# bliunlpr/Robust_e2e_gan

Hardware: AMD Instinct MI355X
Metric: joint_train utterances/sec (higher is better)
Workload: dtype f32; 1 GPU; config4: joint_train.py full GAN+ASR step, B=32 per GPU, T=800, F=257->80, L=40, V=4233, enhancer 2xBLSTM-256, VGG+3xBLSTMP-512, loc-attention decoder 300, D basic ndf64, Adadelta; global_batch=32, per_rank_batch=32, parallelism=dp1, utterance_lengths=560..800 frames (mean 680 of T=800)

## Files before the change

### robust_e2e_gan_amd/csrc/wino_wgrad.hip

```cpp
#include <hip/hip_runtime.h>
#include "../../include/re2e.h"
#include "common.h"

namespace {
typedef float f32x16 __attribute__((ext_vector_type(16)));
typedef float f32x2 __attribute__((ext_vector_type(2)));
constexpr unsigned WW_OOB = 0x80000000u;
constexpr int WW_CB = 64, WW_OB = 32;

struct WwArgs {
  const float* x; const float* dy; float* slabs;
  int NI, H, W, C, Cout;
  int px, py, npatch, nsplit, ncb, nblk;
  unsigned x_bytes, dy_bytes;
  const int* row_lim;
  int flat;
  int dbg;
};

template <int TXW>
__global__ __launch_bounds__(256, 2) void wino_wgrad_kernel(WwArgs p) {
  constexpr int TYH = 32 / TXW, PW = 2 * TXW, PH = 2 * TYH;
  constexpr int XW = PW + 2, XH = PH + 2, XPIX = XW * XH;
  constexpr int XIT = (XPIX * 16 + 255) / 256, DIT = PW * PH * 8 / 256;
  extern __shared__ __attribute__((aligned(16))) float smem[];
  float* xs = smem;
  float* ds = smem + XPIX * WW_CB;
  const int tid = threadIdx.x, lane = tid & 63, lr = lane & 31, lh = lane >> 5;
  const int wid = __builtin_amdgcn_readfirstlane(tid >> 6);
  const int xk = blockIdx.x >> 3;
  const int blk = p.flat ? blockIdx.x % p.nblk : xk % p.nblk, split = p.flat ? blockIdx.x / p.nblk : (xk / p.nblk) * 8 + (blockIdx.x & 7);
  if (split >= p.nsplit) return;
  const int cb = blk % p.ncb, ob = blk / p.ncb;
  const int c0 = cb * WW_CB, o0 = ob * WW_OB;
  const __amdgpu_buffer_rsrc_t rsX = __builtin_amdgcn_make_buffer_rsrc(const_cast<float*>(p.x), 0, p.x_bytes, 0x00020000);
  const __amdgpu_buffer_rsrc_t rsD = __builtin_amdgcn_make_buffer_rsrc(const_cast<float*>(p.dy), 0, p.dy_bytes, 0x00020000);
  const int per = (p.npatch + p.nsplit - 1) / p.nsplit;
  const int pbeg = split * per, pend = min(p.npatch, pbeg + per);

  f32x4 xr[XIT], dr[DIT];
  auto load_patch = [&](int pi) {
    const int n = pi / (p.py * p.px), rem = pi - n * (p.py * p.px);
    const int pyi = rem / p.px, pxi = rem - pyi * p.px;
    const int y0 = pyi * PH, x0 = pxi * PW;
#pragma unroll
    for (int it = 0; it < XIT; ++it) {
      const int item = it * 256 + tid, pix = item >> 4, c4 = item & 15;
      const int yy = pix / XW, xx = pix - yy * XW, iy = y0 - 1 + yy, ix = x0 - 1 + xx;
      const bool ok = pix < XPIX && (unsigned)iy < (unsigned)p.H && (unsigned)ix < (unsigned)p.W;
      const unsigned off = (unsigned)((((n * p.H + iy) * p.W + ix) * p.C + c0 + c4 * 4) * 4);
      xr[it] = __builtin_bit_cast(f32x4, __builtin_amdgcn_raw_buffer_load_b128(rsX, ok ? off : WW_OOB, 0, 0));
    }
#pragma unroll
    for (int it = 0; it < DIT; ++it) {
      const int item = it * 256 + tid, pix = item >> 3, o4 = item & 7;
      const int yy = pix / PW, xx = pix - yy * PW, oy = y0 + yy, ox = x0 + xx;
      const bool ok = oy < p.H && ox < p.W;
      const unsigned off = (unsigned)((((n * p.H + oy) * p.W + ox) * p.Cout + o0 + o4 * 4) * 4);
      dr[it] = __builtin_bit_cast(f32x4, __builtin_amdgcn_raw_buffer_load_b128(rsD, ok ? off : WW_OOB, 0, 0));
    }
  };
  auto store_patch = [&]() {
#pragma unroll
    for (int it = 0; it < XIT; ++it) {
      const int item = it * 256 + tid;
      if (item < XPIX * 16) *reinterpret_cast<f32x4*>(xs + item * 4) = xr[it];
    }
#pragma unroll
    for (int it = 0; it < DIT; ++it) *reinterpret_cast<f32x4*>(ds + (it * 256 + tid) * 4) = dr[it];
  };

  const int rA = wid == 0 ? 0 : (wid == 2 ? 2 : 1), rB = wid == 3 ? 3 : (wid == 2 ? 1 : 2);
  const float sg = wid == 1 ? 1.f : -1.f;
  const float a0 = wid == 3 ? 0.f : 1.f, a1 = wid == 0 ? 0.f : (wid == 1 ? 1.f : -1.f);
  constexpr int HR = TYH / 2;
  const float* xA = xs + ((rA + 2 * HR * lh) * XW) * WW_CB + 2 * lr;
  const float* xB = xs + ((rB + 2 * HR * lh) * XW) * WW_CB + 2 * lr;
  const float* dB = ds + (2 * HR * lh * PW) * WW_OB + lr;

  f32x16 acc[4][2];
#pragma unroll
  for (int j = 0; j < 4; ++j)
#pragma unroll
    for (int ct = 0; ct < 2; ++ct)
#pragma unroll
      for (int r = 0; r < 16; ++r) acc[j][ct][r] = 0.f;

  for (int pi = pbeg; pi < pend; ++pi) {
    if (p.row_lim) {
      const int n = pi / (p.py * p.px), pyi = (pi - n * (p.py * p.px)) / p.px;
      if (pyi * PH >= p.row_lim[n]) continue;
    }
    load_patch(pi);
    store_patch();
    __syncthreads();
    f32x2 t[4], v[2][4];
    float m[2][4];
    auto prep = [&](const int s, f32x2 (&vv)[4], float (&mm)[4]) {
      const int tyl = s / TXW, txl = s % TXW;
#pragma unroll
      for (int j = 0; j < 4; ++j) {
        if (txl != 0 && j < 2) { t[j] = t[j + 2]; continue; }
        const f32x2 da = *reinterpret_cast<const f32x2*>(xA + ((2 * tyl) * XW + 2 * txl + j) * WW_CB);
        const f32x2 db = *reinterpret_cast<const f32x2*>(xB + ((2 * tyl) * XW + 2 * txl + j) * WW_CB);
        t[j] = da + sg * db;
      }
      vv[0] = t[0] - t[2]; vv[1] = t[1] + t[2]; vv[2] = t[2] - t[1]; vv[3] = t[1] - t[3];
      const float e00 = dB[((2 * tyl) * PW + 2 * txl) * WW_OB], e01 = dB[((2 * tyl) * PW + 2 * txl + 1) * WW_OB];
      const float e10 = dB[((2 * tyl + 1) * PW + 2 * txl) * WW_OB], e11 = dB[((2 * tyl + 1) * PW + 2 * txl + 1) * WW_OB];
      const float s0 = a0 * e00 + a1 * e10, s1 = a0 * e01 + a1 * e11;
      mm[0] = s0; mm[1] = s0 + s1; mm[2] = s0 - s1; mm[3] = -s1;
    };
    prep(0, v[0], m[0]);
#pragma unroll
    for (int s = 0; s < 16; ++s) {
      if (s + 1 < 16) prep(s + 1, v[(s + 1) & 1], m[(s + 1) & 1]);
#pragma unroll
      for (int j = 0; j < 4; ++j) {
        acc[j][0] = __builtin_amdgcn_mfma_f32_32x32x2f32(v[s & 1][j][0], m[s & 1][j], acc[j][0], 0, 0, 0);
        acc[j][1] = __builtin_amdgcn_mfma_f32_32x32x2f32(v[s & 1][j][1], m[s & 1][j], acc[j][1], 0, 0, 0);
      }
      if (s + 1 < 16) {
#pragma unroll
        for (int g = 0; g < 8; ++g) {
          __builtin_amdgcn_sched_group_barrier(0x008, 1, 0);
          __builtin_amdgcn_sched_group_barrier(0x100, 1, 0);
          __builtin_amdgcn_sched_group_barrier(0x002, 4, 0);
        }
      }
    }
    __syncthreads();
  }
  float* sl = p.slabs + ((long)split * 16 + 4 * wid) * p.C * p.Cout;
#pragma unroll
  for (int j = 0; j < 4; ++j)
#pragma unroll
    for (int ct = 0; ct < 2; ++ct)
#pragma unroll
      for (int r = 0; r < 16; ++r) {
        const int c = c0 + 2 * ((r & 3) + 8 * (r >> 2) + 4 * lh) + ct;
        sl[((long)j * p.C + c) * p.Cout + o0 + lr] = acc[j][ct][r];
      }
}

#ifdef RE2E_EXPERIMENTS
#include "experiments/wino_wgrad_dma.hip"
#endif

__global__ __launch_bounds__(1024) void wino_wgrad_reduce_kernel(const float* __restrict__ slabs, int nsplit, long tot, float* __restrict__ red) {
  __shared__ float part[16][64];
  const int e = threadIdx.x & 63, sl = threadIdx.x >> 6;
  const long i = (long)blockIdx.x * 64 + e;
  float s = 0.f;
  if (i < tot)
    for (int z = sl; z < nsplit; z += 16) s += slabs[(long)z * tot + i];
  part[sl][e] = s;
  __syncthreads();
  if (sl != 0 || i >= tot) return;
  s = 0.f;
#pragma unroll
  for (int q = 0; q < 16; ++q) s += part[q][e];
  red[i] = s;
}

__global__ __launch_bounds__(256) void wino_wgrad_final_kernel(const float* __restrict__ slabs, int nsplit, int C, int Cout, float* __restrict__ gw,
                                                               float beta) {
  const long i = (long)blockIdx.x * 256 + threadIdx.x;
  const long CO = (long)C * Cout;
  if (i >= CO) return;
  const int o = (int)(i % Cout), c = (int)(i / Cout);
  float u[4][4];
#pragma unroll
  for (int pos = 0; pos < 16; ++pos) u[pos >> 2][pos & 3] = 0.f;
  for (int s = 0; s < nsplit; ++s) {
    const float* sp = slabs + (long)s * 16 * CO + i;
#pragma unroll
    for (int pos = 0; pos < 16; ++pos) u[pos >> 2][pos & 3] += sp[pos * CO];
  }
  float t[3][4];
#pragma unroll
  for (int j = 0; j < 4; ++j) {
    t[0][j] = u[0][j] + 0.5f * (u[1][j] + u[2][j]);
    t[1][j] = 0.5f * (u[1][j] - u[2][j]);
    t[2][j] = 0.5f * (u[1][j] + u[2][j]) + u[3][j];
  }
  float* wp = gw + ((long)o * C + c) * 9;
#pragma unroll
  for (int a = 0; a < 3; ++a) {
    const float r0 = t[a][0] + 0.5f * (t[a][1] + t[a][2]), r1 = 0.5f * (t[a][1] - t[a][2]), r2 = 0.5f * (t[a][1] + t[a][2]) + t[a][3];
    if (beta != 0.f) { wp[a * 3] += r0; wp[a * 3 + 1] += r1; wp[a * 3 + 2] += r2; }
    else { wp[a * 3] = r0; wp[a * 3 + 1] = r1; wp[a * 3 + 2] = r2; }
  }
}

struct WwPlan { bool wide; int px, py, npatch, nsplit, ncb, nblk; size_t bytes; };
WwPlan ww_plan(int NI, int H, int W, int C, int Cout) {
  WwPlan q;
  const long pad_w = (long)cdiv(H, 8) * 8 * cdiv(W, 16) * 16, pad_n = (long)cdiv(H, 16) * 16 * cdiv(W, 8) * 8;
  q.wide = pad_w <= pad_n;
  q.px = cdiv(W, q.wide ? 16 : 8); q.py = cdiv(H, q.wide ? 8 : 16);
  q.npatch = NI * q.py * q.px;
  q.ncb = C / WW_CB; q.nblk = q.ncb * (Cout / WW_OB);
  int s = cdiv(1536, q.nblk);
  if (s > q.npatch / 8) s = q.npatch / 8;
  if (s < 1) s = 1;
  q.nsplit = s;
  q.bytes = (size_t)(s + 1) * 16 * C * Cout * sizeof(float);
  return q;
}

template <int TXW>
void launch_ww(const WwArgs& a, hipStream_t st) {
  constexpr int PW = 2 * TXW, PH = 64 / TXW;
#ifdef RE2E_EXPERIMENTS
  static const bool dma = exp_env("RE2E_WW_DMA") && atoi(exp_env("RE2E_WW_DMA")) == 1;
  if (dma) {
    constexpr size_t lds2 = (size_t)2 * (192 * WW_CB + PW * PH * WW_OB) * sizeof(float);
    static LdsLimit lim2;
    lim2.ensure(reinterpret_cast<const void*>(&wino_wgrad_dma_kernel<TXW>), lds2);
    hipLaunchKernelGGL((wino_wgrad_dma_kernel<TXW>), dim3((unsigned)(cdiv(a.nsplit, 8) * 8 * a.nblk)), dim3(256), lds2, st, a);
    return;
  }
#endif
  constexpr size_t lds = (size_t)((PW + 2) * (PH + 2) * WW_CB + PW * PH * WW_OB) * sizeof(float);
  static LdsLimit lim;
  lim.ensure(reinterpret_cast<const void*>(&wino_wgrad_kernel<TXW>), lds);
  hipLaunchKernelGGL((wino_wgrad_kernel<TXW>), dim3((unsigned)(cdiv(a.nsplit, 8) * 8 * a.nblk)), dim3(256), lds, st, a);
}
}

extern "C" size_t re2e_conv3x3_wino_wgrad_workspace_bytes(int NI, int H, int W, int C, int Cout) {
  if (NI <= 0 || H <= 0 || W <= 0 || C <= 0 || Cout <= 0 || C % WW_CB || Cout % WW_OB) return 0;
  return ww_plan(NI, H, W, C, Cout).bytes;
}

static int ww_impl(const float* in, int NI, int H, int W, int C, const float* dout, int Cout, float* gw, float beta, const int* row_lim, void* workspace,
                   size_t workspace_bytes, hipStream_t stream) {
  RE2E_CHECK_ARG(in && dout && gw && workspace, "null operand");
  RE2E_CHECK_ARG(NI > 0 && H > 0 && W > 0 && C > 0 && Cout > 0, "bad geometry");
  RE2E_CHECK_ARG(beta == 0.f || beta == 1.f, "beta must be 0 or 1");
  if (C % WW_CB || Cout % WW_OB) { re2e_set_error("re2e_conv3x3_wino_wgrad: C must be a multiple of 64 and Cout of 32 (got %d, %d)", C, Cout); return RE2E_EUNSUPPORTED; }
  const long x_bytes = (long)NI * H * W * C * 4, dy_bytes = (long)NI * H * W * Cout * 4;
  if (x_bytes >= 0x7FFFFF00L || dy_bytes >= 0x7FFFFF00L) { re2e_set_error("re2e_conv3x3_wino_wgrad: tensors must be < 2 GiB"); return RE2E_EUNSUPPORTED; }
  RE2E_CHECK_ARG((reinterpret_cast<uintptr_t>(in) & 15) == 0 && (reinterpret_cast<uintptr_t>(dout) & 15) == 0, "in / dout must be 16-byte aligned");
  const WwPlan q = ww_plan(NI, H, W, C, Cout);
  RE2E_CHECK_ARG(workspace_bytes >= q.bytes, "workspace too small (re2e_conv3x3_wino_wgrad_workspace_bytes)");
  WwArgs a;
  a.x = in; a.dy = dout; a.slabs = static_cast<float*>(workspace);
  a.NI = NI; a.H = H; a.W = W; a.C = C; a.Cout = Cout;
  a.px = q.px; a.py = q.py; a.npatch = q.npatch; a.nsplit = q.nsplit; a.ncb = q.ncb; a.nblk = q.nblk;
  a.x_bytes = (unsigned)x_bytes; a.dy_bytes = (unsigned)dy_bytes;
  a.row_lim = row_lim;
  a.dbg = exp_env("RE2E_WW_DBG") ? atoi(exp_env("RE2E_WW_DBG")) : 0;
  a.flat = exp_env("RE2E_WW_FLAT") ? atoi(exp_env("RE2E_WW_FLAT")) : 0;
  static const bool log_calls = getenv("RE2E_IGEMM_LOG") != nullptr;
  if (log_calls)
    fprintf(stderr, "[igemm] A=WinoW B=DenseM tile=64x32x2 vec=1 M=%d N=%d K=%ld splits=%d\n", 9 * C, Cout, (long)NI * H * W, q.nsplit);
  if (q.wide) launch_ww<8>(a, stream); else launch_ww<4>(a, stream);
  const long tot = 16L * C * Cout;
  float* red = a.slabs + (long)q.nsplit * tot;
  hipLaunchKernelGGL(wino_wgrad_reduce_kernel, dim3((unsigned)cdiv(tot, 64)), dim3(1024), 0, stream, a.slabs, q.nsplit, tot, red);
  hipLaunchKernelGGL(wino_wgrad_final_kernel, dim3((unsigned)cdiv((long)C * Cout, 256)), dim3(256), 0, stream, red, 1, C, Cout, gw, beta);
  RE2E_LAUNCH_CHECK();
  return RE2E_OK;
}

extern "C" int re2e_conv3x3_wino_wgrad(const float* in, int NI, int H, int W, int C, const float* dout, int Cout, float* gw, float beta, void* workspace,
                                       size_t workspace_bytes, hipStream_t stream) {
  return ww_impl(in, NI, H, W, C, dout, Cout, gw, beta, nullptr, workspace, workspace_bytes, stream);
}

extern "C" int re2e_conv3x3_wino_wgrad_rows(const float* in, int NI, int H, int W, int C, const float* dout, int Cout, float* gw, float beta,
                                            const int* row_lim, void* workspace, size_t workspace_bytes, hipStream_t stream) {
  RE2E_CHECK_ARG(row_lim, "null row limits");
  return ww_impl(in, NI, H, W, C, dout, Cout, gw, beta, row_lim, workspace, workspace_bytes, stream);
}
```

Baseline: 686.9 utterances/s.

## Widen Winograd wgrad tile to two output blocks, balance valid patches, fuse reductions

The Winograd weight-gradient kernel now gives each block two 32-wide output-channel blocks (NOB=2). This reuses the transformed input across twice the MFMAs and adds register prefetch of the next patch into the main loop. Split ranges are now computed over valid patches only, following the row limits, so padded rows no longer leave splits unbalanced. The separate reduce and final kernels are merged into one finish kernel, and slab stores use buffer stores. The cost is more register pressure: occupancy bound drops to one block per SIMD, and the split-count heuristic changes.

```diff
diff --git a/robust_e2e_gan_amd/csrc/experiments/wino_wgrad_deep.hip b/robust_e2e_gan_amd/csrc/experiments/wino_wgrad_deep.hip
--- /dev/null
+++ b/robust_e2e_gan_amd/csrc/experiments/wino_wgrad_deep.hip
@@ -0,0 +1,61 @@
+template <int TXW, int NOB>
+__device__ __forceinline__ void ww_products_deep(const float* xA, const float* xB, const float* dB, const float sg, const float a0, const float a1,
+                                                 f32x16 (&acc)[NOB][4][2]) {
+  constexpr int TYH = 32 / TXW, PW = 2 * TXW, XW = PW + 2, OBW = WW_OB * NOB;
+  f32x2 t[4], v[2][4];
+  float m[2][NOB][4];
+  struct Raw { f32x2 a[4], b[4]; float e[NOB][4]; };
+  auto fetch = [&](const int s, Raw& w) {
+    const int tyl = s / TXW, txl = s % TXW;
+#pragma unroll
+    for (int j = 0; j < 4; ++j) {
+      if (txl != 0 && j < 2) continue;
+      w.a[j] = *reinterpret_cast<const f32x2*>(xA + ((2 * tyl) * XW + 2 * txl + j) * WW_CB);
+      w.b[j] = *reinterpret_cast<const f32x2*>(xB + ((2 * tyl) * XW + 2 * txl + j) * WW_CB);
+    }
+#pragma unroll
+    for (int nb = 0; nb < NOB; ++nb) {
+      const float* dn = dB + nb * WW_OB;
+      w.e[nb][0] = dn[((2 * tyl) * PW + 2 * txl) * OBW]; w.e[nb][1] = dn[((2 * tyl) * PW + 2 * txl + 1) * OBW];
+      w.e[nb][2] = dn[((2 * tyl + 1) * PW + 2 * txl) * OBW]; w.e[nb][3] = dn[((2 * tyl + 1) * PW + 2 * txl + 1) * OBW];
+    }
+  };
+  auto xform = [&](const int s, const Raw& w, f32x2 (&vv)[4], float (&mm)[NOB][4]) {
+    const int txl = s % TXW;
+#pragma unroll
+    for (int j = 0; j < 4; ++j) {
+      if (txl != 0 && j < 2) { t[j] = t[j + 2]; continue; }
+      t[j] = w.a[j] + sg * w.b[j];
+    }
+    vv[0] = t[0] - t[2]; vv[1] = t[1] + t[2]; vv[2] = t[2] - t[1]; vv[3] = t[1] - t[3];
+#pragma unroll
+    for (int nb = 0; nb < NOB; ++nb) {
+      const float s0 = a0 * w.e[nb][0] + a1 * w.e[nb][2], s1 = a0 * w.e[nb][1] + a1 * w.e[nb][3];
+      mm[nb][0] = s0; mm[nb][1] = s0 + s1; mm[nb][2] = s0 - s1; mm[nb][3] = -s1;
+    }
+  };
+  Raw w[2];
+  fetch(0, w[0]);
+  fetch(1, w[1]);
+  xform(0, w[0], v[0], m[0]);
+#pragma unroll
+  for (int s = 0; s < 16; ++s) {
+    if (s + 1 < 16) xform(s + 1, w[(s + 1) & 1], v[(s + 1) & 1], m[(s + 1) & 1]);
+    if (s + 2 < 16) fetch(s + 2, w[s & 1]);
+#pragma unroll
+    for (int j = 0; j < 4; ++j)
+#pragma unroll
+      for (int nb = 0; nb < NOB; ++nb) {
+        acc[nb][j][0] = __builtin_amdgcn_mfma_f32_32x32x2f32(v[s & 1][j][0], m[s & 1][nb][j], acc[nb][j][0], 0, 0, 0);
+        acc[nb][j][1] = __builtin_amdgcn_mfma_f32_32x32x2f32(v[s & 1][j][1], m[s & 1][nb][j], acc[nb][j][1], 0, 0, 0);
+      }
+    if (s + 1 < 16) {
+#pragma unroll
+      for (int g = 0; g < 8 * NOB; ++g) {
+        __builtin_amdgcn_sched_group_barrier(0x008, 1, 0);
+        __builtin_amdgcn_sched_group_barrier(0x100, 1, 0);
+        __builtin_amdgcn_sched_group_barrier(0x002, NOB == 1 ? 4 : 2, 0);
+      }
+    }
+  }
+}
diff --git a/robust_e2e_gan_amd/csrc/wino_wgrad.hip b/robust_e2e_gan_amd/csrc/wino_wgrad.hip
--- a/robust_e2e_gan_amd/csrc/wino_wgrad.hip
+++ b/robust_e2e_gan_amd/csrc/wino_wgrad.hip
@@ -1,6 +1,7 @@
 #include <hip/hip_runtime.h>
 #include "../../include/re2e.h"
 #include "common.h"
+#include "ww_ranges.h"
 
 namespace {
 typedef float f32x16 __attribute__((ext_vector_type(16)));
@@ -18,44 +19,51 @@
   int dbg;
 };
 
-template <int TXW>
-__global__ __launch_bounds__(256, 2) void wino_wgrad_kernel(WwArgs p) {
+#ifdef RE2E_EXPERIMENTS
+#include "experiments/wino_wgrad_deep.hip"
+#endif
+
+template <int TXW, int NOB, bool DEEP = false>
+__global__ __launch_bounds__(256, NOB == 1 ? 2 : 1) void wino_wgrad_kernel(WwArgs p) {
   constexpr int TYH = 32 / TXW, PW = 2 * TXW, PH = 2 * TYH;
   constexpr int XW = PW + 2, XH = PH + 2, XPIX = XW * XH;
-  constexpr int XIT = (XPIX * 16 + 255) / 256, DIT = PW * PH * 8 / 256;
+  constexpr int OBW = WW_OB * NOB;
+  constexpr int XIT = (XPIX * 16 + 255) / 256, DIT = PW * PH * (OBW / 4) / 256;
+  constexpr bool PF = NOB > 1;
   extern __shared__ __attribute__((aligned(16))) float smem[];
   float* xs = smem;
   float* ds = smem + XPIX * WW_CB;
   const int tid = threadIdx.x, lane = tid & 63, lr = lane & 31, lh = lane >> 5;
   const int wid = __builtin_amdgcn_readfirstlane(tid >> 6);
-  const int xk = blockIdx.x >> 3;
-  const int blk = p.flat ? blockIdx.x % p.nblk : xk % p.nblk, split = p.flat ? blockIdx.x / p.nblk : (xk / p.nblk) * 8 + (blockIdx.x & 7);
+  int blk, split;
+  ww_block((int)blockIdx.x, p.nblk, &blk, &split);
   if (split >= p.nsplit) return;
   const int cb = blk % p.ncb, ob = blk / p.ncb;
-  const int c0 = cb * WW_CB, o0 = ob * WW_OB;
+  const int c0 = cb * WW_CB, o0 = ob * OBW;
   const __amdgpu_buffer_rsrc_t rsX = __builtin_amdgcn_make_buffer_rsrc(const_cast<float*>(p.x), 0, p.x_bytes, 0x00020000);
   const __amdgpu_buffer_rsrc_t rsD = __builtin_amdgcn_make_buffer_rsrc(const_cast<float*>(p.dy), 0, p.dy_bytes, 0x00020000);
-  const int per = (p.npatch + p.nsplit - 1) / p.nsplit;
-  const int pbeg = split * per, pend = min(p.npatch, pbeg + per);
+  long vbeg, vend;
+  ww_range(ww_total(p.row_lim, p.NI, p.H, PH, p.py, p.px), p.nsplit, split, &vbeg, &vend);
+  WwCursor cur = ww_seek(p.row_lim, p.NI, p.H, PH, p.py, p.px, vbeg);
 
   f32x4 xr[XIT], dr[DIT];
-  auto load_patch = [&](int pi) {
-    const int n = pi / (p.py * p.px), rem = pi - n * (p.py * p.px);
-    const int pyi = rem / p.px, pxi = rem - pyi * p.px;
+  auto load_patch = [&](const WwCursor& q) {
+    const int n = q.n, pyi = q.r / p.px, pxi = q.r - pyi * p.px;
     const int y0 = pyi * PH, x0 = pxi * PW;
+    const int lim = p.row_lim ? min(max(p.row_lim[n], 0), p.H) : p.H, xlim = min(lim + 1, p.H);
 #pragma unroll
     for (int it = 0; it < XIT; ++it) {
       const int item = it * 256 + tid, pix = item >> 4, c4 = item & 15;
       const int yy = pix / XW, xx = pix - yy * XW, iy = y0 - 1 + yy, ix = x0 - 1 + xx;
-      const bool ok = pix < XPIX && (unsigned)iy < (unsigned)p.H && (unsigned)ix < (unsigned)p.W;
+      const bool ok = pix < XPIX && (unsigned)iy < (unsigned)xlim && (unsigned)ix < (unsigned)p.W;
       const unsigned off = (unsigned)((((n * p.H + iy) * p.W + ix) * p.C + c0 + c4 * 4) * 4);
       xr[it] = __builtin_bit_cast(f32x4, __builtin_amdgcn_raw_buffer_load_b128(rsX, ok ? off : WW_OOB, 0, 0));
     }
 #pragma unroll
     for (int it = 0; it < DIT; ++it) {
-      const int item = it * 256 + tid, pix = item >> 3, o4 = item & 7;
+      const int item = it * 256 + tid, pix = item / (OBW / 4), o4 = item % (OBW / 4);
       const int yy = pix / PW, xx = pix - yy * PW, oy = y0 + yy, ox = x0 + xx;
-      const bool ok = oy < p.H && ox < p.W;
+      const bool ok = oy < lim && ox < p.W;
       const unsigned off = (unsigned)((((n * p.H + oy) * p.W + ox) * p.Cout + o0 + o4 * 4) * 4);
       dr[it] = __builtin_bit_cast(f32x4, __builtin_amdgcn_raw_buffer_load_b128(rsD, ok ? off : WW_OOB, 0, 0));
     }
@@ -76,27 +84,37 @@
   constexpr int HR = TYH / 2;
   const float* xA = xs + ((rA + 2 * HR * lh) * XW) * WW_CB + 2 * lr;
   const float* xB = xs + ((rB + 2 * HR * lh) * XW) * WW_CB + 2 * lr;
-  const float* dB = ds + (2 * HR * lh * PW) * WW_OB + lr;
-
-  f32x16 acc[4][2];
-#pragma unroll
-  for (int j = 0; j < 4; ++j)
-#pragma unroll
-    for (int ct = 0; ct < 2; ++ct)
-#pragma unroll
-      for (int r = 0; r < 16; ++r) acc[j][ct][r] = 0.f;
-
-  for (int pi = pbeg; pi < pend; ++pi) {
-    if (p.row_lim) {
-      const int n = pi / (p.py * p.px), pyi = (pi - n * (p.py * p.px)) / p.px;
-      if (pyi * PH >= p.row_lim[n]) continue;
-    }
-    load_patch(pi);
+  const float* dB = ds + (2 * HR * lh * PW) * OBW + lr;
+
+  f32x16 acc[NOB][4][2];
+#pragma unroll
+  for (int nb = 0; nb < NOB; ++nb)
+#pragma unroll
+    for (int j = 0; j < 4; ++j)
+#pragma unroll
+      for (int ct = 0; ct < 2; ++ct)
+#pragma unroll
+        for (int r = 0; r < 16; ++r) acc[nb][j][ct][r] = 0.f;
+
+  if (PF && vbeg < vend) load_patch(cur);
+  for (long k = vbeg; k < vend; ++k) {
+    if (!PF) load_patch(cur);
     store_patch();
     __syncthreads();
+    if (k + 1 < vend) {
+      ww_next(&cur, p.row_lim, p.NI, p.H, PH, p.py, p.px);
+      if (PF) load_patch(cur);
+    }
+#ifdef RE2E_EXPERIMENTS
+    if constexpr (DEEP) {
+      ww_products_deep<TXW, NOB>(xA, xB, dB, sg, a0, a1, acc);
+      __syncthreads();
+      continue;
+    }
+#endif
     f32x2 t[4], v[2][4];
-    float m[2][4];
-    auto prep = [&](const int s, f32x2 (&vv)[4], float (&mm)[4]) {
+    float m[2][NOB][4];
+    auto prep = [&](const int s, f32x2 (&vv)[4], float (&mm)[NOB][4]) {
       const int tyl = s / TXW, txl = s % TXW;
 #pragma unroll
       for (int j = 0; j < 4; ++j) {
@@ -106,83 +124,93 @@
         t[j] = da + sg * db;
       }
       vv[0] = t[0] - t[2]; vv[1] = t[1] + t[2]; vv[2] = t[2] - t[1]; vv[3] = t[1] - t[3];
-      const float e00 = dB[((2 * tyl) * PW + 2 * txl) * WW_OB], e01 = dB[((2 * tyl) * PW + 2 * txl + 1) * WW_OB];
-      const float e10 = dB[((2 * tyl + 1) * PW + 2 * txl) * WW_OB], e11 = dB[((2 * tyl + 1) * PW + 2 * txl + 1) * WW_OB];
-      const float s0 = a0 * e00 + a1 * e10, s1 = a0 * e01 + a1 * e11;
-      mm[0] = s0; mm[1] = s0 + s1; mm[2] = s0 - s1; mm[3] = -s1;
+#pragma unroll
+      for (int nb = 0; nb < NOB; ++nb) {
+        const float* dn = dB + nb * WW_OB;
+        const float e00 = dn[((2 * tyl) * PW + 2 * txl) * OBW], e01 = dn[((2 * tyl) * PW + 2 * txl + 1) * OBW];
+        const float e10 = dn[((2 * tyl + 1) * PW + 2 * txl) * OBW], e11 = dn[((2 * tyl + 1) * PW + 2 * txl + 1) * OBW];
+        const float s0 = a0 * e00 + a1 * e10, s1 = a0 * e01 + a1 * e11;
+        mm[nb][0] = s0; mm[nb][1] = s0 + s1; mm[nb][2] = s0 - s1; mm[nb][3] = -s1;
+      }
     };
     prep(0, v[0], m[0]);
 #pragma unroll
     for (int s = 0; s < 16; ++s) {
       if (s + 1 < 16) prep(s + 1, v[(s + 1) & 1], m[(s + 1) & 1]);
 #pragma unroll
-      for (int j = 0; j < 4; ++j) {
-        acc[j][0] = __builtin_amdgcn_mfma_f32_32x32x2f32(v[s & 1][j][0], m[s & 1][j], acc[j][0], 0, 0, 0);
-        acc[j][1] = __builtin_amdgcn_mfma_f32_32x32x2f32(v[s & 1][j][1], m[s & 1][j], acc[j][1], 0, 0, 0);
-      }
+      for (int j = 0; j < 4; ++j)
+#pragma unroll
+        for (int nb = 0; nb < NOB; ++nb) {
+          acc[nb][j][0] = __builtin_amdgcn_mfma_f32_32x32x2f32(v[s & 1][j][0], m[s & 1][nb][j], acc[nb][j][0], 0, 0, 0);
+          acc[nb][j][1] = __builtin_amdgcn_mfma_f32_32x32x2f32(v[s & 1][j][1], m[s & 1][nb][j], acc[nb][j][1], 0, 0, 0);
+        }
       if (s + 1 < 16) {
 #pragma unroll
-        for (int g = 0; g < 8; ++g) {
+        for (int g = 0; g < 8 * NOB; ++g) {
           __builtin_amdgcn_sched_group_barrier(0x008, 1, 0);
           __builtin_amdgcn_sched_group_barrier(0x100, 1, 0);
-          __builtin_amdgcn_sched_group_barrier(0x002, 4, 0);
+          __builtin_amdgcn_sched_group_barrier(0x002, NOB == 1 ? 4 : 2, 0);
         }
       }
     }
     __syncthreads();
   }
-  float* sl = p.slabs + ((long)split * 16 + 4 * wid) * p.C * p.Cout;
-#pragma unroll
-  for (int j = 0; j < 4; ++j)
-#pragma unroll
-    for (int ct = 0; ct < 2; ++ct)
-#pragma unroll
-      for (int r = 0; r < 16; ++r) {
-        const int c = c0 + 2 * ((r & 3) + 8 * (r >> 2) + 4 * lh) + ct;
-        sl[((long)j * p.C + c) * p.Cout + o0 + lr] = acc[j][ct][r];
-      }
+  const unsigned slab_bytes = 16u * p.C * p.Cout * 4u;
+  const __amdgpu_buffer_rsrc_t rsS = __builtin_amdgcn_make_buffer_rsrc(p.slabs + (long)split * 16 * p.C * p.Cout, 0, slab_bytes, 0x00020000);
+  const int lane_off = (((4 * wid * p.C) + c0 + 8 * lh) * p.Cout + o0 + lr) * 4;
+#pragma unroll
+  for (int nb = 0; nb < NOB; ++nb)
+#pragma unroll
+    for (int j = 0; j < 4; ++j)
+#pragma unroll
+      for (int ct = 0; ct < 2; ++ct)
+#pragma unroll
+        for (int r = 0; r < 16; ++r) {
+          const int uni = ((j * p.C + 2 * ((r & 3) + 8 * (r >> 2)) + ct) * p.Cout + nb * WW_OB) * 4;
+          const float val = acc[nb][j][ct][r];
+          __builtin_amdgcn_raw_buffer_store_b32(__builtin_bit_cast(unsigned, val), rsS, lane_off, uni, 0);
+        }
 }
 
 #ifdef RE2E_EXPERIMENTS
 #include "experiments/wino_wgrad_dma.hip"
 #endif
 
-__global__ __launch_bounds__(1024) void wino_wgrad_reduce_kernel(const float* __restrict__ slabs, int nsplit, long tot, float* __restrict__ red) {
-  __shared__ float part[16][64];
-  const int e = threadIdx.x & 63, sl = threadIdx.x >> 6;
-  const long i = (long)blockIdx.x * 64 + e;
-  float s = 0.f;
-  if (i < tot)
-    for (int z = sl; z < nsplit; z += 16) s += slabs[(long)z * tot + i];
-  part[sl][e] = s;
+constexpr int WF_E = 32, WF_L = 32;
+__global__ __launch_bounds__(WF_E * WF_L) void wino_wgrad_finish_kernel(const float* __restrict__ slabs, int nsplit, int C, int Cout, float* __restrict__ gw,
+                                                                        float beta) {
+  __shared__ float part[WF_L][16][WF_E];
+  const int e = threadIdx.x & (WF_E - 1), sl = threadIdx.x / WF_E;
+  const long CO = (long)C * Cout, i = (long)blockIdx.x * WF_E + e;
+  float u[16];
+#pragma unroll
+  for (int pos = 0; pos < 16; ++pos) u[pos] = 0.f;
+  if (i < CO)
+    for (int z = sl; z < nsplit; z += WF_L) {
+      const float* sp = slabs + (long)z * 16 * CO + i;
+#pragma unroll
+      for (int pos = 0; pos < 16; ++pos) u[pos] += sp[pos * CO];
+    }
+#pragma unroll
+  for (int pos = 0; pos < 16; ++pos) part[sl][pos][e] = u[pos];
   __syncthreads();
-  if (sl != 0 || i >= tot) return;
-  s = 0.f;
-#pragma unroll
-  for (int q = 0; q < 16; ++q) s += part[q][e];
-  red[i] = s;
-}
-
-__global__ __launch_bounds__(256) void wino_wgrad_final_kernel(const float* __restrict__ slabs, int nsplit, int C, int Cout, float* __restrict__ gw,
-                                                               float beta) {
-  const long i = (long)blockIdx.x * 256 + threadIdx.x;
-  const long CO = (long)C * Cout;
-  if (i >= CO) return;
+  if (threadIdx.x < 16 * WF_E) {
+    const int pos = threadIdx.x / WF_E;
+    float s = 0.f;
+#pragma unroll
+    for (int q = 0; q < WF_L; ++q) s += part[q][pos][e];
+    part[0][pos][e] = s;
+  }
+  __syncthreads();
+  if (threadIdx.x >= WF_E || i >= CO) return;
   const int o = (int)(i % Cout), c = (int)(i / Cout);
-  float u[4][4];
-#pragma unroll
-  for (int pos = 0; pos < 16; ++pos) u[pos >> 2][pos & 3] = 0.f;
-  for (int s = 0; s < nsplit; ++s) {
-    const float* sp = slabs + (long)s * 16 * CO + i;
-#pragma unroll
-    for (int pos = 0; pos < 16; ++pos) u[pos >> 2][pos & 3] += sp[pos * CO];
-  }
   float t[3][4];
 #pragma unroll
   for (int j = 0; j < 4; ++j) {
-    t[0][j] = u[0][j] + 0.5f * (u[1][j] + u[2][j]);
-    t[1][j] = 0.5f * (u[1][j] - u[2][j]);
-    t[2][j] = 0.5f * (u[1][j] + u[2][j]) + u[3][j];
+    const float u0 = part[0][j][e], u1 = part[0][4 + j][e], u2 = part[0][8 + j][e], u3 = part[0][12 + j][e];
+    t[0][j] = u0 + 0.5f * (u1 + u2);
+    t[1][j] = 0.5f * (u1 - u2);
+    t[2][j] = 0.5f * (u1 + u2) + u3;
   }
   float* wp = gw + ((long)o * C + c) * 9;
 #pragma unroll
@@ -193,39 +221,48 @@
   }
 }
 
-struct WwPlan { bool wide; int px, py, npatch, nsplit, ncb, nblk; size_t bytes; };
+struct WwPlan { bool wide; int nob, px, py, npatch, nsplit, ncb, nblk; size_t bytes; };
 WwPlan ww_plan(int NI, int H, int W, int C, int Cout) {
   WwPlan q;
+  static const int nob_max = exp_env("RE2E_WW_NOB") ? atoi(exp_env("RE2E_WW_NOB")) : 2;
+  static const bool dma = exp_env("RE2E_WW_DMA") && atoi(exp_env("RE2E_WW_DMA")) == 1;
   const long pad_w = (long)cdiv(H, 8) * 8 * cdiv(W, 16) * 16, pad_n = (long)cdiv(H, 16) * 16 * cdiv(W, 8) * 8;
   q.wide = pad_w <= pad_n;
   q.px = cdiv(W, q.wide ? 16 : 8); q.py = cdiv(H, q.wide ? 8 : 16);
   q.npatch = NI * q.py * q.px;
-  q.ncb = C / WW_CB; q.nblk = q.ncb * (Cout / WW_OB);
-  int s = cdiv(1536, q.nblk);
-  if (s > q.npatch / 8) s = q.npatch / 8;
-  if (s < 1) s = 1;
-  q.nsplit = s;
-  q.bytes = (size_t)(s + 1) * 16 * C * Cout * sizeof(float);
+  q.nob = nob_max >= 2 && !dma && Cout % (2 * WW_OB) == 0 ? 2 : 1;
+  q.ncb = C / WW_CB; q.nblk = q.ncb * (Cout / (WW_OB * q.nob));
+  q.nsplit = ww_plan_nsplit(q.npatch, q.nblk, q.nob == 2 ? 256 : 512);
+  q.bytes = (size_t)q.nsplit * 16 * C * Cout * sizeof(float);
   return q;
 }
 
-template <int TXW>
+template <int TXW, int NOB>
 void launch_ww(const WwArgs& a, hipStream_t st) {
   constexpr int PW = 2 * TXW, PH = 64 / TXW;
 #ifdef RE2E_EXPERIMENTS
   static const bool dma = exp_env("RE2E_WW_DMA") && atoi(exp_env("RE2E_WW_DMA")) == 1;
-  if (dma) {
+  if (dma && NOB == 1) {
     constexpr size_t lds2 = (size_t)2 * (192 * WW_CB + PW * PH * WW_OB) * sizeof(float);
     static LdsLimit lim2;
     lim2.ensure(reinterpret_cast<const void*>(&wino_wgrad_dma_kernel<TXW>), lds2);
-    hipLaunchKernelGGL((wino_wgrad_dma_kernel<TXW>), dim3((unsigned)(cdiv(a.nsplit, 8) * 8 * a.nblk)), dim3(256), lds2, st, a);
+    hipLaunchKernelGGL((wino_wgrad_dma_kernel<TXW>), dim3((unsigned)ww_grid(a.nsplit, a.nblk)), dim3(256), lds2, st, a);
     return;
   }
 #endif
-  constexpr size_t lds = (size_t)((PW + 2) * (PH + 2) * WW_CB + PW * PH * WW_OB) * sizeof(float);
+  constexpr size_t lds = (size_t)((PW + 2) * (PH + 2) * WW_CB + PW * PH * WW_OB * NOB) * sizeof(float);
   static LdsLimit lim;
-  lim.ensure(reinterpret_cast<const void*>(&wino_wgrad_kernel<TXW>), lds);
-  hipLaunchKernelGGL((wino_wgrad_kernel<TXW>), dim3((unsigned)(cdiv(a.nsplit, 8) * 8 * a.nblk)), dim3(256), lds, st, a);
+#ifdef RE2E_EXPERIMENTS
+  static const bool deep = exp_env("RE2E_WW_DEEP") && atoi(exp_env("RE2E_WW_DEEP")) == 1;
+  if constexpr (NOB == 2) if (deep) {
+    static LdsLimit lim3;
+    lim3.ensure(reinterpret_cast<const void*>(&wino_wgrad_kernel<TXW, NOB, true>), lds);
+    hipLaunchKernelGGL((wino_wgrad_kernel<TXW, NOB, true>), dim3((unsigned)ww_grid(a.nsplit, a.nblk)), dim3(256), lds, st, a);
+    return;
+  }
+#endif
+  lim.ensure(reinterpret_cast<const void*>(&wino_wgrad_kernel<TXW, NOB>), lds);
+  hipLaunchKernelGGL((wino_wgrad_kernel<TXW, NOB>), dim3((unsigned)ww_grid(a.nsplit, a.nblk)), dim3(256), lds, st, a);
 }
 }
 
@@ -255,12 +292,10 @@
   a.flat = exp_env("RE2E_WW_FLAT") ? atoi(exp_env("RE2E_WW_FLAT")) : 0;
   static const bool log_calls = getenv("RE2E_IGEMM_LOG") != nullptr;
   if (log_calls)
-    fprintf(stderr, "[igemm] A=WinoW B=DenseM tile=64x32x2 vec=1 M=%d N=%d K=%ld splits=%d\n", 9 * C, Cout, (long)NI * H * W, q.nsplit);
-  if (q.wide) launch_ww<8>(a, stream); else launch_ww<4>(a, stream);
-  const long tot = 16L * C * Cout;
-  float* red = a.slabs + (long)q.nsplit * tot;
-  hipLaunchKernelGGL(wino_wgrad_reduce_kernel, dim3((unsigned)cdiv(tot, 64)), dim3(1024), 0, stream, a.slabs, q.nsplit, tot, red);
-  hipLaunchKernelGGL(wino_wgrad_final_kernel, dim3((unsigned)cdiv((long)C * Cout, 256)), dim3(256), 0, stream, red, 1, C, Cout, gw, beta);
+    fprintf(stderr, "[igemm] A=WinoW B=DenseM tile=64x%dx2 vec=1 M=%d N=%d K=%ld splits=%d\n", WW_OB * q.nob, 9 * C, Cout, (long)NI * H * W, q.nsplit);
+  if (q.nob == 2) { if (q.wide) launch_ww<8, 2>(a, stream); else launch_ww<4, 2>(a, stream); }
+  else { if (q.wide) launch_ww<8, 1>(a, stream); else launch_ww<4, 1>(a, stream); }
+  hipLaunchKernelGGL(wino_wgrad_finish_kernel, dim3((unsigned)cdiv((long)C * Cout, WF_E)), dim3(WF_E * WF_L), 0, stream, a.slabs, q.nsplit, C, Cout, gw, beta);
   RE2E_LAUNCH_CHECK();
   return RE2E_OK;
 }
diff --git a/robust_e2e_gan_amd/csrc/ww_ranges.h b/robust_e2e_gan_amd/csrc/ww_ranges.h
--- /dev/null
+++ b/robust_e2e_gan_amd/csrc/ww_ranges.h
@@ -0,0 +1,73 @@
+#pragma once
+
+#if defined(__HIPCC__) || defined(__CUDACC__)
+#define WW_HD __host__ __device__ inline
+#else
+#define WW_HD inline
+#endif
+
+WW_HD int ww_valid_rows(int lim, int H, int PH, int py) {
+  if (lim <= 0) return 0;
+  if (lim > H) lim = H;
+  const int r = (lim + PH - 1) / PH;
+  return r < py ? r : py;
+}
+
+WW_HD int ww_plan_nsplit(int npatch, int nblk, int resident) {
+  int s = resident / nblk;
+  if (s > npatch / 8) s = npatch / 8;
+  s &= ~7;
+  return s < 8 ? 8 : s;
+}
+
+WW_HD int ww_grid(int nsplit, int nblk) { return ((nsplit + 7) / 8) * 8 * nblk; }
+
+WW_HD void ww_block(int bid, int nblk, int* blk, int* split) {
+  const int xk = bid >> 3;
+  *blk = xk % nblk;
+  *split = (xk / nblk) * 8 + (bid & 7);
+}
+
+WW_HD void ww_range(long V, int nsplit, int split, long* beg, long* end) {
+  *beg = V * split / nsplit;
+  *end = V * (split + 1) / nsplit;
+}
+
+struct WwCursor { int n, r, cnt; };
+
+WW_HD int ww_image_patches(const int* row_lim, int n, int H, int PH, int py, int px) {
+  return (row_lim ? ww_valid_rows(row_lim[n], H, PH, py) : py) * px;
+}
+
+WW_HD long ww_total(const int* row_lim, int NI, int H, int PH, int py, int px) {
+  if (!row_lim) return (long)NI * py * px;
+  long v = 0;
+  for (int n = 0; n < NI; ++n) v += ww_image_patches(row_lim, n, H, PH, py, px);
+  return v;
+}
+
+WW_HD WwCursor ww_seek(const int* row_lim, int NI, int H, int PH, int py, int px, long v) {
+  WwCursor c;
+  if (!row_lim) {
+    c.cnt = py * px; c.n = (int)(v / c.cnt); c.r = (int)(v - (long)c.n * c.cnt);
+    return c;
+  }
+  long cum = 0, before = 0;
+  int n0 = 0;
+  for (int n = 0; n < NI; ++n) {
+    cum += ww_image_patches(row_lim, n, H, PH, py, px);
+    if (cum <= v) { n0 = n + 1; before = cum; }
+  }
+  c.n = n0; c.r = (int)(v - before);
+  c.cnt = n0 < NI ? ww_image_patches(row_lim, n0, H, PH, py, px) : 0;
+  return c;
+}
+
+WW_HD void ww_next(WwCursor* c, const int* row_lim, int NI, int H, int PH, int py, int px) {
+  if (++c->r < c->cnt) return;
+  c->r = 0;
+  do {
+    ++c->n;
+    c->cnt = c->n < NI ? ww_image_patches(row_lim, c->n, H, PH, py, px) : 1;
+  } while (c->cnt == 0);
+}
```

Result: no change. 688.3 utterances/s (median of 6 runs) (+0.2%).
